# alshai/rowbowt

Hardware: AMD Instinct MI355X
Metric: reads/s (100 bp, count+locate) (higher is better)
Workload: dtype u32/u64

## Files before the change

### rowbowt_amd/csrc/k_runs.hip

```cpp
#include <type_traits>

#include "rbg_runs2_device.hpp"
#include "rbg_jump.h"

namespace rbg {
namespace {

struct PackedBits {
    const uint4 *__restrict__ cp;
    uint4 w;
    uint32_t widx, navail;
    uint64_t sr;
    __device__ __forceinline__ uint32_t next_word() {
        if (widx == 4) { w = *cp++; widx = 0; }
        const uint32_t v = w.x;
        w.x = w.y; w.y = w.z; w.z = w.w;
        ++widx;
        return v;
    }
    __device__ __forceinline__ uint32_t take(uint32_t nb) {
        if (navail < nb) { sr |= static_cast<uint64_t>(next_word()) << navail; navail += 32; }
        const uint32_t v = static_cast<uint32_t>(sr & ((uint64_t(1) << nb) - 1));
        sr >>= nb;
        navail -= nb;
        return v;
    }
};

template <bool GLDS>
__device__ __forceinline__ bool jump_probe_wave(const void *__restrict__ tab, const uint64_t nb, const bool probing, const JumpKey &key, uint32_t v[3],
                                                uint32_t &buckets, lds_byte *tile) {
    uint32_t state = probing ? kJumpNext : kJumpAbsent;
    uint64_t b = probing ? jump_home(jump_hash(key), nb) : 0u;
    uint64_t left = nb;
    while (__ballot(state == kJumpNext)) {
        const bool undecided = state == kJumpNext;
        uint32_t w[16];
        quad_fetch_issue<GLDS>(reinterpret_cast<uint64_t>(tab) + (undecided ? b : 0u) * kJumpBucketBytes, w, tile);
        quad_fetch_take<GLDS>(w, tile);
        if (undecided) {
            ++buckets;
            state = jump_bucket(w, key, v);
            b = jump_next(b, nb);
            if (--left == 0 && state == kJumpNext) state = kJumpAbsent;
        }
    }
    return state <= kJumpHit1;
}

template <typename P, bool TOEHOLD, bool PACKED = false, bool STATS = false, bool GLDS = false, bool STAGE = false>
__global__ __launch_bounds__(512, STATS ? 2 : 4) void k_find_range_runs(const DevIndex ix, const void *__restrict__ src_a,
                                                        const void *__restrict__ src_b, const uint64_t N,
                                                        uint64_t *__restrict__ lo_out, uint64_t *__restrict__ hi_out,
                                                        uint64_t *__restrict__ ss_out, unsigned long long *__restrict__ stats,
                                                        const uint32_t *__restrict__ sel, const uint32_t *__restrict__ nsel) {
    const uint64_t Neff = sel ? static_cast<uint64_t>(*nsel) : N;
    const uint8_t *__restrict__ seqs = static_cast<const uint8_t *>(src_a);
    const uint64_t *__restrict__ off = static_cast<const uint64_t *>(src_b);
    const uint4 *__restrict__ chunks = static_cast<const uint4 *>(src_a);
    const uint2 *__restrict__ meta = static_cast<const uint2 *>(src_b);
    __shared__ uint8_t s_lut[256];
    __shared__ uint8_t s_lut2[256];
    __shared__ uint8_t s_mslot[4];
    __shared__ __align__(16) unsigned char s_tile[GLDS ? 8 * kTileBytes : 16];
    __shared__ uint32_t s_codes[STAGE ? 8 * kStageWords * 64 : 1];
    for (int t = threadIdx.x; t < 256; t += blockDim.x) {
        s_lut[t] = ix.lut[t];
        s_lut2[t] = ix.nmajor ? ix.lut2[t] : 0xFFu;
    }
    RBG_RUN_SEARCH2_SHARED;
    const RunSearch2<P> S2 = stage_run_search2<P>(ix, s_tab_first, s_ent2, s_dir2, s_rec2, s_dyn);
    const uint32_t *tab_first = s_tab_first;
    lds_byte *tile = (lds_byte *)s_tile + (GLDS ? (threadIdx.x >> 6) * kTileBytes : 0u);
    if (PACKED || STAGE) {
        for (int t = threadIdx.x; t < 256; t += blockDim.x)
            if (s_lut2[t] != 0xFFu) s_mslot[s_lut2[t] & 3u] = s_lut[t];
        __syncthreads();
    }
    const uint32_t D = ix.run_ksteps, DMASK = ix.run_depth_mask | 1u;
    const uint32_t M = ix.nmajor;
    const uint32_t lane = threadIdx.x & (kWave - 1);
    lds_u32 *codes = (lds_u32 *)s_codes + (STAGE ? (threadIdx.x >> 6) * (kStageWords * 64u) + lane : 0u);
    const StageTab stage_tab{ix.stage_code[0], ix.stage_code[1], ix.stage_byte[0], ix.stage_byte[1], ix.stage_shift};
    const bool stage_on = STAGE && ix.stage_ok != 0 && M == 4;

    unsigned long long c_occ = 0, c_reads = 0;
    uint32_t c_matched = 0;
    unsigned long long st[kStatSearchN] = {0, 0, 0, 0, 0, 0, 0, 0};
    const uint64_t stride = static_cast<uint64_t>(gridDim.x) * blockDim.x;
    const uint64_t wave_first = static_cast<uint64_t>(blockIdx.x) * blockDim.x + (threadIdx.x & ~(kWave - 1));
    for (uint64_t base = wave_first; base < Neff; base += stride) {
        bool valid = base + lane < Neff;
        const uint64_t i = (sel && valid) ? static_cast<uint64_t>(sel[base + lane]) : base + lane;
        uint64_t beg = 0, p = 0;
        PackedBits bs{chunks, make_uint4(0, 0, 0, 0), 4u, 0u, 0ull};
        if (PACKED) {
            if (valid) {
                const uint2 mt = meta[i];
                if (mt.y & 0x80000000u) valid = false;
                else { p = mt.y; bs.cp = chunks + mt.x; }
            }
        } else if (valid) { beg = off[i]; p = off[i + 1]; }
        bool staged = false;
        if constexpr (STAGE && !PACKED) {
            if (stage_on && __ballot(valid && p - beg > kStageCap) == 0) {
                uint32_t nch = 0;
                const bool bad = valid && stage_read(reinterpret_cast<const uint4 *>(seqs), beg, p, stage_tab, codes, nch);
                if (STATS) st[kStChunks] += nch;
                staged = __ballot(bad) == 0;
                if (staged) { p -= beg; beg = 0; }
                else if (STATS) st[kStChunks] -= nch;
            }
        }
        auto walk = [&](auto staged_tag) __attribute__((always_inline)) {
            constexpr bool STAGED = decltype(staged_tag)::value;
            const uint64_t p_end = p;
            uint64_t p_min = p;
            const uint32_t m32 = static_cast<uint32_t>(p);
            uint64_t lo = 0, hi = ix.n - 1;
            uint64_t k = TOEHOLD ? ix.last_run_sample : 0;
            bool alive = valid;
            bool pend = false;
            uint32_t pend_d = 0, pend_rec = 0;
            uint64_t pend_e = 0;
            ByteCursor rd{reinterpret_cast<const uint4 *>(seqs), ~uint64_t(0), make_uint4(0, 0, 0, 0)};
            bool jumped = false;
            if constexpr (STAGED && sizeof(P) == 4) {
                if (ix.jump) {
                    const bool probing = valid && m32 >= ix.jump_k;
                    JumpKey key{{codes[0], codes[64], codes[128], codes[192]}};
                    jump_key_mask(key, ix.jump_k);
                    uint32_t v[3] = {0, 0, 0}, nbk = 0;
                    if (jump_probe_wave<GLDS>(ix.jump, ix.jump_buckets, probing, key, v, nbk, tile)) {
                        lo = v[0]; hi = v[1];
                        if (TOEHOLD) k = v[2] == 0xFFFFFFFFu ? ~uint64_t(0) : static_cast<uint64_t>(v[2]);
                        p -= ix.jump_k;
                        jumped = true;
                        if (STATS) st[kStSymbols] += ix.jump_k;
                    }
                    if (STATS) st[kStFtab] += nbk;
                }
            }
            if (!jumped && valid && ix.ftab_k && p - beg >= ix.ftab_k) {
                uint64_t idx = 0;
                bool all_major = true;
                PackedBits probe = bs;
                if constexpr (STAGED) {
                    const uint32_t w0 = codes[0];
                    idx = ix.ftab_k >= 16u ? w0 : (w0 & ((1u << (2u * ix.ftab_k)) - 1u));
                } else if (PACKED) {
                    idx = probe.take(2 * ix.ftab_k);
                } else {
                    uint64_t pw = 1;
                    for (uint32_t t = 1; t <= ix.ftab_k; ++t) {
                        const uint32_t mm = s_lut2[rd.at(p - t)];
                        all_major = all_major && mm != 0xFFu;
                        idx += (mm & 3u) * pw;
                        pw *= M;
                    }
                }
                uint64_t flo, fhi2, fk;
                if (STATS) { if (!STAGED) p_min = p - ix.ftab_k; if (all_major) st[kStFtab] += 1; }
                if (all_major && ftab_lookup<P>(ix, idx, flo, fhi2, fk)) {
                    if (PACKED) bs = probe;
                    lo = flo; hi = fhi2;
                    if (TOEHOLD) k = fk;
                    p -= ix.ftab_k;
                    if (STATS) st[kStSymbols] += ix.ftab_k;
                    if (hi < lo) { alive = false; p = beg; }
                }
            }
            struct Pick { uint32_t d, adv, rec; bool ok; };
            auto pick_at = [&](const uint64_t pp) __attribute__((always_inline)) -> Pick {
                Pick s{0u, 1u, 0u, true};
                if constexpr (STAGED) {
                    s.adv = pp < D ? static_cast<uint32_t>(pp) : D;
                    s.adv = 32u - static_cast<uint32_t>(__clz(DMASK & ((2u << (s.adv - 1)) - 1u)));
                    const uint32_t t0 = m32 - static_cast<uint32_t>(pp);
                    const lds_u32 *cw = codes + (t0 >> 4) * 64u;
                    const uint32_t v = __builtin_amdgcn_alignbit(cw[64], cw[0], (t0 & 15u) * 2u) & ((1u << (2u * s.adv)) - 1u);
                    s.rec = run_record(tab_first, s.adv, s.adv == 1 ? static_cast<uint32_t>(s_mslot[v]) : v);
                    s.d = s.adv - 1;
                } else if (PACKED) {
                    s.adv = pp < D ? static_cast<uint32_t>(pp) : D;
                    s.adv = 32u - static_cast<uint32_t>(__clz(DMASK & ((2u << (s.adv - 1)) - 1u)));
                    const uint32_t v = bs.take(2 * s.adv);
                    s.rec = run_record(tab_first, s.adv, s.adv == 1 ? static_cast<uint32_t>(s_mslot[v]) : v);
                    s.d = s.adv - 1;
                } else {
                    const uint64_t q = pp - 1;
                    const uint32_t c = rd.at(q);
                    if (STATS && q < p_min) p_min = q;
                    const uint32_t m0 = s_lut2[c];
                    uint32_t acc = m0;
                    if (m0 != 0xFFu) {
                        uint32_t pw = M, run_acc = m0;
    #pragma unroll 1
                        for (uint32_t t = 1; t < static_cast<uint32_t>(kMaxRunDepth); ++t) {
                            if (t >= D || q < beg + t) break;
                            const uint32_t mm = s_lut2[rd.at(q - t)];
                            if (STATS && q - t < p_min) p_min = q - t;
                            if (mm == 0xFFu) break;
                            run_acc += mm * pw;
                            pw *= M;
                            if ((DMASK >> t) & 1u) { s.adv = t + 1; acc = run_acc; }
                        }
                    }
                    if (s.adv == 1) {
                        const uint32_t slot = s_lut[c];
                        if (slot == 0xFFu || slot >= static_cast<uint32_t>(kLdsSyms)) s.ok = false;
                        else s.rec = run_record(tab_first, 1u, slot);
                    } else {
                        s.d = s.adv - 1;
                        s.rec = run_record(tab_first, s.adv, acc);
                    }
                }
                return s;
            };
            constexpr bool AHEAD = !PACKED || STAGED;
            Pick cur{0u, 1u, 0u, false};
            RunHot Rcur{0, 0};
            if (AHEAD && alive && p > beg) {
                cur = pick_at(p);
                if (cur.ok) Rcur = load_run_tab<P>(S2, cur.d, cur.rec);
            }
            while (__ballot(alive && p > beg)) {
                bool stepping = alive && p > beg;
                if (!AHEAD && stepping) {
                    cur = pick_at(p);
                    if (cur.ok) Rcur = load_run_tab<P>(S2, cur.d, cur.rec);
                }
                if (stepping && !cur.ok) { alive = false; stepping = false; }
                const uint32_t d = cur.d, adv = cur.adv, rec = cur.rec;
                const RunHot R = Rcur;
                const uint64_t p_next = p - adv;
                if (AHEAD && stepping && p_next > beg) {
                    cur = pick_at(p_next);
                    if (cur.ok) Rcur = load_run_tab<P>(S2, cur.d, cur.rec);
                }
                RunStep r;
                lane_lf2_quad<P, STATS, false, GLDS>(S2, stepping, d, rec, R, lo, hi + 1, r, st, tile);
                if (stepping) {
                    if (STATS) st[kStSymbols] += adv;
                    const uint64_t c_inside = r.c_upto - r.c_before;
                    if (c_inside == 0) {
                        alive = false;
                    } else {
                        if (TOEHOLD) {
                            if (r.inside) k = k - adv;
                            else { pend = true; pend_d = d; pend_rec = rec; pend_e = r.samp_e; k = 0; }
                        }
                        lo = r.F + r.c_before;
                        hi = lo + c_inside - 1;
                        p = p_next;
                    }
                }
            }
            if (TOEHOLD && alive && pend) {
                k += run_step_sample2<P>(ix, S2, pend_d, pend_rec, pend_e);
                if (STATS) st[kStResample] += 1;
            }
            if (STATS && !PACKED && !STAGED && p_end > p_min) st[kStChunks] += ((p_end - 1) >> 4) - (p_min >> 4) + 1;
            if (STATS && PACKED && valid) st[kStChunks] += (p_end + 63) >> 6;
            if (!alive) { lo = 1; hi = 0; k = 0; }
            if (valid) {
                lo_out[i] = lo;
                hi_out[i] = hi;
                if (TOEHOLD) ss_out[i] = k;
                c_reads += 1;
                if (alive) { c_matched += 1; c_occ += hi - lo + 1; }
            }
        };
        if (STAGE && staged) walk(std::integral_constant<bool, STAGE>{}); else walk(std::false_type{});
    }
    c_reads = wave_sum(c_reads);
    const unsigned long long w_matched = wave_sum(static_cast<unsigned long long>(c_matched));
    c_occ = wave_sum(c_occ);
    if (lane == 0 && c_reads) {
        atomicAdd(&ix.counters[0], c_reads);
        if (w_matched) atomicAdd(&ix.counters[1], w_matched);
        if (c_occ) atomicAdd(&ix.counters[2], c_occ);
    }
    if (STATS) {
#pragma unroll
        for (int t = 0; t < kStatSearchN; ++t) {
            const unsigned long long v = wave_sum(st[t]);
            if (lane == 0 && v) atomicAdd(&stats[t], v);
        }
    }
}

template <typename P> struct ChunkR { static constexpr int v = 8; };
__device__ __forceinline__ uint64_t locus_toehold_r(const DevIndex &ix, const uint64_t key, const uint64_t *__restrict__ k, const uint64_t i) {
    if (key == ~uint64_t(0)) return k[i];
    const uint32_t low = ix.order_lowbits, db = ix.order_dbits;
    const uint64_t doc = (key >> low) & ((uint64_t(1) << db) - 1u);
    return ix.order_docs[doc] + (((key >> (db + low)) << low) | (key & ((uint64_t(1) << low) - 1u)));
}

template <typename P, typename OUT = uint64_t, bool STATS = false, bool SUB = false, bool HI8 = false>
__global__ __launch_bounds__(256, 4) void k_locate_fill_runs2(const DevIndex ix, const uint64_t *__restrict__ lo,
                                                          const uint64_t *__restrict__ hi, const uint64_t *__restrict__ k,
                                                          const uint64_t N, const uint64_t max_hits,
                                                          const uint64_t *__restrict__ loc_off, OUT *__restrict__ locs,
                                                          const uint64_t *__restrict__ sub, const uint32_t *__restrict__ order,
                                                          const uint64_t *__restrict__ skeys, unsigned long long *__restrict__ stats) {
    constexpr int kChunkR = ChunkR<P>::v;
    constexpr bool RING = true;
    using Stage = ChainStage<P, kChunkR, SUB, RING, HI8>;
    __shared__ Stage S;
    const uint64_t out_elem0 = reinterpret_cast<uintptr_t>(locs) / sizeof(OUT);
    const int wv = threadIdx.x >> 6, lane = threadIdx.x & (kWave - 1);
    unsigned long long c_locs = 0;
    unsigned long long st_phi = 0, st_ent = 0, st_chains = 0;
    const uint64_t n = ix.n;
    const uint64_t stride = static_cast<uint64_t>(gridDim.x) * blockDim.x;
    for (uint64_t base = static_cast<uint64_t>(blockIdx.x) * blockDim.x + wv * kWave; base < N; base += stride) {
        const uint64_t j = base + lane;
        uint64_t i = j;
        if (order && j < N) i = order[j];
        uint64_t occ = 0, k1 = 0, dst = 0;
        if (i < N && j < N) {
            dst = loc_off[i];
            if (skeys) {
                if (ix.order_docs) k1 = locus_toehold_r(ix, skeys[j], k, i);
                else if (sizeof(P) == 4) { const uint32_t k32 = reinterpret_cast<const uint32_t *>(skeys)[j]; k1 = k32 == 0xFFFFFFFFu ? k[i] : k32; }
                else k1 = skeys[j];
                occ = loc_off[i + 1] - dst;
            } else {
                const uint64_t l = lo[i], h = hi[i];
                occ = h >= l ? h - l + 1 : 0;
                if (occ > max_hits) occ = max_hits;
                k1 = k[i];
            }
        }
        const uint64_t minus = (SUB && i < N && j < N) ? sub[i] : 0;
        const uint32_t a = (RING && occ) ? static_cast<uint32_t>((out_elem0 + dst) & static_cast<uint64_t>(kChunkR - 1)) : 0u;
        S.dst[wv][lane] = dst - a;
        if (SUB) S.minus[wv][lane] = minus;
        const bool off_text = Stage::kSentinel && k1 >= n;
        if (off_text && occ) locs[dst] = static_cast<OUT>(k1 - minus);
        c_locs += occ;
        if (STATS && occ) st_chains += 1;
        uint64_t wmax = occ + a;
#pragma unroll
        for (int o = kWave / 2; o > 0; o >>= 1) {
            const uint64_t other = __shfl_xor(wmax, o, kWave);
            wmax = other > wmax ? other : wmax;
        }
        for (uint64_t t0 = 0; t0 < wmax; t0 += kChunkR) {
            const uint32_t cnt = chain_round_count<kChunkR>(occ, t0);
            S.bounds[wv][lane] = chain_window_bounds<kChunkR>(occ, a, t0);
#pragma unroll 1
            for (int e = 0; e < kChunkR; ++e) {
                const bool mine = static_cast<uint32_t>(e) < cnt;
                if (mine && (e || t0)) {
                    uint64_t s;
                    if (k1 >= n) {
                        s = (ix.phi_last_base + (k1 - ix.phi_last_pos)) % n;
                    } else {
                        bool found;
                        uint64_t val;
                        uint32_t ents, rounds;
                        lane_phi<P>(ix, k1, found, val, ents, rounds);
                        if (STATS) { st_phi += 1; st_ent += ents + 7u * rounds; }
                        s = found ? val : ix.phi_last_base + k1 + 1;
                        if (s >= n) s -= n;
                    }
                    k1 = s;
                }
                if (mine) chain_put(S, wv, lane, a + static_cast<uint32_t>(t0) + e, k1, e == 0 && t0 == 0 && off_text);
            }
            wave_lds_sync();
            chain_flush(S, wv, lane, t0, locs);
            wave_lds_sync();
        }
        wave_lds_sync();
    }
    c_locs = wave_sum(c_locs);
    if (lane == 0 && c_locs) atomicAdd(&ix.counters[3], c_locs);
    if (STATS) {
        st_phi = wave_sum(st_phi);
        st_ent = wave_sum(st_ent);
        st_chains = wave_sum(st_chains);
        if (lane == 0) {
            if (st_phi) atomicAdd(&stats[kLsPhiSteps], st_phi);
            if (st_ent) atomicAdd(&stats[kLsPhiOvf], st_ent);
            if (st_chains) atomicAdd(&stats[kLsChains], st_chains);
            if (c_locs) atomicAdd(&stats[kLsLocs], c_locs);
        }
    }
}

}

int launch_find_range_runs_impl(const DevIndex &ix, const LaunchCfg &cfg, const void *src_a, const void *src_b, uint64_t N,
                                uint64_t *lo, uint64_t *hi, uint64_t *ssamp, void *stream, bool packed, unsigned long long *stats,
                                const uint32_t *sel = nullptr, const uint32_t *nsel = nullptr) {
    if (N == 0) return 0;
    hipStream_t st = static_cast<hipStream_t>(stream);
    const size_t lds = run_search2_lds(ix);
    static const bool glds = [] { const char *e = std::getenv("RBG_REC_FETCH"); return !(e && std::strcmp(e, "quad") == 0); }();
    static const bool stage = [] { const char *e = std::getenv("RBG_STAGE_READS"); return !(e && e[0] == '0'); }();
    LaunchCfg c = cfg;
    c.block_threads = 512;
    c.max_blocks = cfg.max_blocks > 0 ? std::max(1, cfg.max_blocks / 2) : 256 * 16;
    const dim3 grid(sel ? std::min(grid_for(c, N), 256) : grid_for(c, N)), block(512);
#define RBG_LAUNCH_FRR1(PT, TOE, PK, STS, GL, SG)                                                      \
    do {                                                                                               \
        auto kern = k_find_range_runs<PT, TOE, PK, STS, GL, SG>;                                       \
        raise_lds(kern, lds, (GL ? 8 * kTileBytes : 0) + (SG ? 8 * kStageWaveBytes : 0));             \
        hipLaunchKernelGGL(kern, grid, block, lds, st, ix, src_a, src_b, N, lo, hi, ssamp, stats, sel, nsel);     \
    } while (0)
#define RBG_LAUNCH_FRR(PT, TOE, PK, STS)                                                               \
    do {                                                                                               \
        if (glds && stage && !PK && !sel) RBG_LAUNCH_FRR1(PT, TOE, false, STS, true, true);            \
        else if (glds) RBG_LAUNCH_FRR1(PT, TOE, PK, STS, true, false);                                 \
        else RBG_LAUNCH_FRR1(PT, TOE, PK, STS, false, false);                                          \
    } while (0)
#define RBG_LAUNCH_FRR2(PT, TOE)                                                                       \
    do {                                                                                               \
        if (stats) { if (packed) return static_cast<int>(hipErrorNotSupported); RBG_LAUNCH_FRR(PT, TOE, false, true); } \
        else if (packed) RBG_LAUNCH_FRR(PT, TOE, true, false);                                         \
        else RBG_LAUNCH_FRR(PT, TOE, false, false);                                                    \
    } while (0)
    if (ix.pos_bytes == 4) {
        if (ssamp) RBG_LAUNCH_FRR2(uint32_t, true); else RBG_LAUNCH_FRR2(uint32_t, false);
    } else {
        if (ssamp) RBG_LAUNCH_FRR2(uint64_t, true); else RBG_LAUNCH_FRR2(uint64_t, false);
    }
#undef RBG_LAUNCH_FRR2
#undef RBG_LAUNCH_FRR
#undef RBG_LAUNCH_FRR1
    return static_cast<int>(hipGetLastError());
}

int launch_find_range_runs(const DevIndex &ix, const LaunchCfg &cfg, const uint8_t *seqs, const uint64_t *off, uint64_t N,
                           uint64_t *lo, uint64_t *hi, uint64_t *ssamp, void *stream, unsigned long long *stats) {
    return launch_find_range_runs_impl(ix, cfg, seqs, off, N, lo, hi, ssamp, stream, false, stats);
}

int launch_find_range_runs_sel(const DevIndex &ix, const LaunchCfg &cfg, const uint8_t *seqs, const uint64_t *off, uint64_t N, uint64_t *lo,
                               uint64_t *hi, uint64_t *ssamp, const uint32_t *sel, const uint32_t *nsel, void *stream) {
    return launch_find_range_runs_impl(ix, cfg, seqs, off, N, lo, hi, ssamp, stream, false, nullptr, sel, nsel);
}

int launch_find_range_runs_packed(const DevIndex &ix, const LaunchCfg &cfg, const uint2 *meta, const uint4 *chunks, uint64_t N,
                                  uint64_t *lo, uint64_t *hi, uint64_t *ssamp, void *stream) {
    return launch_find_range_runs_impl(ix, cfg, chunks, meta, N, lo, hi, ssamp, stream, true, nullptr);
}

int launch_locate_fill_runs(const DevIndex &ix, const LaunchCfg &cfg, const uint64_t *lo, const uint64_t *hi, const uint64_t *k,
                            uint64_t N, uint64_t max_hits, const uint64_t *loc_off, uint64_t *locs, const uint64_t *sub,
                            const void *order, const uint64_t *skeys, void *stream, unsigned long long *stats, uint32_t *locs32) {
    if (N == 0) return 0;
    if ((stats || locs32) && sub) return static_cast<int>(hipErrorInvalidValue);
    hipStream_t st = static_cast<hipStream_t>(stream);
    const dim3 grid(grid_for(cfg, N)), block(256);
    const uint32_t *perm = static_cast<const uint32_t *>(order);
    const bool hi8 = ix.pos_bytes == 8 && ix.n < kChainHi8Limit && chain_hi8_enabled();
#define RBG_LAUNCH_LFR2(PT, OUT, STS, SB, DST) \
    do { \
        if (sizeof(PT) == 8 && hi8) hipLaunchKernelGGL((k_locate_fill_runs2<PT, OUT, STS, SB, sizeof(PT) == 8>), grid, block, 0, st, ix, lo, hi, k, N, max_hits, loc_off, DST, sub, perm, skeys, stats); \
        else hipLaunchKernelGGL((k_locate_fill_runs2<PT, OUT, STS, SB, false>), grid, block, 0, st, ix, lo, hi, k, N, max_hits, loc_off, DST, sub, perm, skeys, stats); \
    } while (0)
    if (locs32) {
        if (ix.pos_bytes != 4) return static_cast<int>(hipErrorInvalidValue);
        RBG_LAUNCH_LFR2(uint32_t, uint32_t, false, false, locs32);
    } else if (stats) {
        if (ix.pos_bytes == 4) RBG_LAUNCH_LFR2(uint32_t, uint64_t, true, false, locs); else RBG_LAUNCH_LFR2(uint64_t, uint64_t, true, false, locs);
    } else if (sub) {
        if (ix.pos_bytes == 4) RBG_LAUNCH_LFR2(uint32_t, uint64_t, false, true, locs); else RBG_LAUNCH_LFR2(uint64_t, uint64_t, false, true, locs);
    } else if (ix.pos_bytes == 4) {
        RBG_LAUNCH_LFR2(uint32_t, uint64_t, false, false, locs);
    } else {
        RBG_LAUNCH_LFR2(uint64_t, uint64_t, false, false, locs);
    }
#undef RBG_LAUNCH_LFR2
    return static_cast<int>(hipGetLastError());
}

}
```

Before: 2.192 billion.

## Park jump-table misses and finish them in a compacted tail kernel

Reads whose jump-table probe misses are no longer walked inside the main wave. They are marked in lo_out, and a second kernel scans the output, compacts the parked read indices into per-wave LDS queues, and walks them with full waves. This targets divergence, where a few slow reads stall a whole wave of fast jump hits. The cost is an extra launch and a full scan of lo_out, and the tail kernel runs smaller blocks at lower occupancy.

```diff
diff --git a/rowbowt_amd/csrc/k_runs.hip b/rowbowt_amd/csrc/k_runs.hip
--- a/rowbowt_amd/csrc/k_runs.hip
+++ b/rowbowt_amd/csrc/k_runs.hip
@@ -2,6 +2,7 @@
 
 #include "rbg_runs2_device.hpp"
 #include "rbg_jump.h"
+#include "rbg_park.h"
 
 namespace rbg {
 namespace {
@@ -48,12 +49,15 @@
     return state <= kJumpHit1;
 }
 
-template <typename P, bool TOEHOLD, bool PACKED = false, bool STATS = false, bool GLDS = false, bool STAGE = false>
-__global__ __launch_bounds__(512, STATS ? 2 : 4) void k_find_range_runs(const DevIndex ix, const void *__restrict__ src_a,
+template <typename P, bool TOEHOLD, bool PACKED = false, bool STATS = false, bool GLDS = false, bool STAGE = false, bool TAIL = false>
+__global__ __launch_bounds__(TAIL ? 256 : 512, TAIL ? (STATS ? 2 : 3) : (STATS ? 2 : 4)) void k_find_range_runs(const DevIndex ix, const void *__restrict__ src_a,
                                                         const void *__restrict__ src_b, const uint64_t N,
                                                         uint64_t *__restrict__ lo_out, uint64_t *__restrict__ hi_out,
                                                         uint64_t *__restrict__ ss_out, unsigned long long *__restrict__ stats,
-                                                        const uint32_t *__restrict__ sel, const uint32_t *__restrict__ nsel) {
+                                                        const uint32_t *__restrict__ sel, const uint32_t *__restrict__ nsel,
+                                                        const uint32_t park) {
+    static_assert(!TAIL || (STAGE && GLDS && !PACKED && sizeof(P) == 4), "the tail walks staged reads of an index with 4-byte positions");
+    constexpr uint32_t kWavesWG = TAIL ? 4 : 8;
     const uint64_t Neff = sel ? static_cast<uint64_t>(*nsel) : N;
     const uint8_t *__restrict__ seqs = static_cast<const uint8_t *>(src_a);
     const uint64_t *__restrict__ off = static_cast<const uint64_t *>(src_b);
@@ -62,8 +66,9 @@
     __shared__ uint8_t s_lut[256];
     __shared__ uint8_t s_lut2[256];
     __shared__ uint8_t s_mslot[4];
-    __shared__ __align__(16) unsigned char s_tile[GLDS ? 8 * kTileBytes : 16];
-    __shared__ uint32_t s_codes[STAGE ? 8 * kStageWords * 64 : 1];
+    __shared__ __align__(16) unsigned char s_tile[GLDS ? kWavesWG * kTileBytes : 16];
+    __shared__ uint32_t s_codes[STAGE ? kWavesWG * kStageWords * 64 : 1];
+    __shared__ uint32_t s_queue[TAIL ? kWavesWG * kParkQueueWords : 1];
     for (int t = threadIdx.x; t < 256; t += blockDim.x) {
         s_lut[t] = ix.lut[t];
         s_lut2[t] = ix.nmajor ? ix.lut2[t] : 0xFFu;
@@ -89,9 +94,7 @@
     unsigned long long st[kStatSearchN] = {0, 0, 0, 0, 0, 0, 0, 0};
     const uint64_t stride = static_cast<uint64_t>(gridDim.x) * blockDim.x;
     const uint64_t wave_first = static_cast<uint64_t>(blockIdx.x) * blockDim.x + (threadIdx.x & ~(kWave - 1));
-    for (uint64_t base = wave_first; base < Neff; base += stride) {
-        bool valid = base + lane < Neff;
-        const uint64_t i = (sel && valid) ? static_cast<uint64_t>(sel[base + lane]) : base + lane;
+    auto iter = [&](bool valid, const uint64_t i) __attribute__((always_inline)) {
         uint64_t beg = 0, p = 0;
         PackedBits bs{chunks, make_uint4(0, 0, 0, 0), 4u, 0u, 0ull};
         if (PACKED) {
@@ -106,10 +109,10 @@
             if (stage_on && __ballot(valid && p - beg > kStageCap) == 0) {
                 uint32_t nch = 0;
                 const bool bad = valid && stage_read(reinterpret_cast<const uint4 *>(seqs), beg, p, stage_tab, codes, nch);
-                if (STATS) st[kStChunks] += nch;
+                if (STATS && !TAIL) st[kStChunks] += nch;
                 staged = __ballot(bad) == 0;
                 if (staged) { p -= beg; beg = 0; }
-                else if (STATS) st[kStChunks] -= nch;
+                else if (STATS && !TAIL) st[kStChunks] -= nch;
             }
         }
         auto walk = [&](auto staged_tag) __attribute__((always_inline)) {
@@ -124,8 +127,8 @@
             uint32_t pend_d = 0, pend_rec = 0;
             uint64_t pend_e = 0;
             ByteCursor rd{reinterpret_cast<const uint4 *>(seqs), ~uint64_t(0), make_uint4(0, 0, 0, 0)};
-            bool jumped = false;
-            if constexpr (STAGED && sizeof(P) == 4) {
+            bool jumped = false, parked = false;
+            if constexpr (STAGED && sizeof(P) == 4 && !TAIL) {
                 if (ix.jump) {
                     const bool probing = valid && m32 >= ix.jump_k;
                     JumpKey key{{codes[0], codes[64], codes[128], codes[192]}};
@@ -137,11 +140,14 @@
                         p -= ix.jump_k;
                         jumped = true;
                         if (STATS) st[kStSymbols] += ix.jump_k;
+                    } else if (park && probing) {
+                        parked = true;
+                        alive = false;
                     }
                     if (STATS) st[kStFtab] += nbk;
                 }
             }
-            if (!jumped && valid && ix.ftab_k && p - beg >= ix.ftab_k) {
+            if (!jumped && !parked && valid && ix.ftab_k && p - beg >= ix.ftab_k) {
                 uint64_t idx = 0;
                 bool all_major = true;
                 PackedBits probe = bs;
@@ -263,7 +269,9 @@
             if (STATS && !PACKED && !STAGED && p_end > p_min) st[kStChunks] += ((p_end - 1) >> 4) - (p_min >> 4) + 1;
             if (STATS && PACKED && valid) st[kStChunks] += (p_end + 63) >> 6;
             if (!alive) { lo = 1; hi = 0; k = 0; }
-            if (valid) {
+            if (parked) {
+                lo_out[i] = kParkMark;
+            } else if (valid) {
                 lo_out[i] = lo;
                 hi_out[i] = hi;
                 if (TOEHOLD) ss_out[i] = k;
@@ -272,6 +280,44 @@
             }
         };
         if (STAGE && staged) walk(std::integral_constant<bool, STAGE>{}); else walk(std::false_type{});
+    };
+    if constexpr (TAIL) {
+        lds_u32 *queue = (lds_u32 *)s_queue + (threadIdx.x >> 6) * kParkQueueWords;
+        const uint64_t W = static_cast<uint64_t>(gridDim.x) * kWavesWG, w = static_cast<uint64_t>(blockIdx.x) * kWavesWG + (threadIdx.x >> 6);
+        const uint64_t r0 = park_first(N, W, w), r1 = park_end(N, W, w);
+        uint64_t pos = r0;
+        uint32_t qn = 0;
+        for (;;) {
+            while (park_scan_more(qn, pos, r1)) {
+                uint64_t v[kParkScanChunks];
+#pragma unroll
+                for (uint32_t c = 0; c < kParkScanChunks; ++c) {
+                    const uint64_t at = pos + c * kParkWave + lane;
+                    v[c] = at < r1 ? lo_out[at] : 0u;
+                }
+#pragma unroll
+                for (uint32_t c = 0; c < kParkScanChunks; ++c) {
+                    const bool marked = v[c] == kParkMark;
+                    const uint64_t mask = __ballot(marked);
+                    if (marked) queue[park_slot(qn, mask, lane)] = static_cast<uint32_t>(pos - r0) + c * kParkWave + lane;
+                    qn += park_count(mask);
+                }
+                pos += kParkScan;
+            }
+            if (qn == 0) break;
+            wave_lds_sync();
+            const uint32_t first = park_take_first(qn);
+            const bool valid = lane < park_take(qn);
+            const uint64_t i = r0 + (valid ? queue[first + lane] : 0u);
+            qn = first;
+            wave_lds_sync();
+            iter(valid, i);
+        }
+    } else {
+        for (uint64_t base = wave_first; base < Neff; base += stride) {
+            const bool valid = base + lane < Neff;
+            iter(valid, (sel && valid) ? static_cast<uint64_t>(sel[base + lane]) : base + lane);
+        }
     }
     c_reads = wave_sum(c_reads);
     const unsigned long long w_matched = wave_sum(static_cast<unsigned long long>(c_matched));
@@ -406,15 +452,31 @@
     c.block_threads = 512;
     c.max_blocks = cfg.max_blocks > 0 ? std::max(1, cfg.max_blocks / 2) : 256 * 16;
     const dim3 grid(sel ? std::min(grid_for(c, N), 256) : grid_for(c, N)), block(512);
+    constexpr size_t kTailStatic = 4 * (kTileBytes + kStageWaveBytes + kParkQueueWords * sizeof(uint32_t));
+    const bool tail_fits = lds + kTailStatic + 1024 <= 160 * 1024;
+    const uint32_t park = (!sel && !packed && glds && stage && ix.pos_bytes == 4 && ix.jump && ix.stage_ok && ix.nmajor == 4 &&
+                           N < kParkMaxReads && tail_fits) ? 1u : 0u;
+    const uint64_t tail_cus = cfg.max_blocks > 0 ? std::max(1, cfg.max_blocks / 32) : 256;
+    const uint64_t tail_per_cu = std::min<uint64_t>(3, std::max<uint64_t>(1, 160 * 1024 / (lds + kTailStatic + 1024)));
+    const dim3 tail_grid(static_cast<unsigned>(std::min<uint64_t>(tail_cus * tail_per_cu, (N + 16 * kParkScan - 1) / (16 * kParkScan)))), tail_block(256);
 #define RBG_LAUNCH_FRR1(PT, TOE, PK, STS, GL, SG)                                                      \
     do {                                                                                               \
         auto kern = k_find_range_runs<PT, TOE, PK, STS, GL, SG>;                                       \
         raise_lds(kern, lds, (GL ? 8 * kTileBytes : 0) + (SG ? 8 * kStageWaveBytes : 0));             \
-        hipLaunchKernelGGL(kern, grid, block, lds, st, ix, src_a, src_b, N, lo, hi, ssamp, stats, sel, nsel);     \
+        hipLaunchKernelGGL(kern, grid, block, lds, st, ix, src_a, src_b, N, lo, hi, ssamp, stats, sel, nsel, (SG && sizeof(PT) == 4) ? park : 0u); \
+    } while (0)
+#define RBG_LAUNCH_FRR_TAIL(TOE, STS)                                                                  \
+    do {                                                                                               \
+        auto tail = k_find_range_runs<uint32_t, TOE, false, STS, true, true, true>;                    \
+        raise_lds(tail, lds, kTailStatic);                                                             \
+        hipLaunchKernelGGL(tail, tail_grid, tail_block, lds, st, ix, src_a, src_b, N, lo, hi, ssamp, stats, sel, nsel, 0u); \
     } while (0)
 #define RBG_LAUNCH_FRR(PT, TOE, PK, STS)                                                               \
     do {                                                                                               \
-        if (glds && stage && !PK && !sel) RBG_LAUNCH_FRR1(PT, TOE, false, STS, true, true);            \
+        if (glds && stage && !PK && !sel) {                                                            \
+            RBG_LAUNCH_FRR1(PT, TOE, false, STS, true, true);                                          \
+            if (sizeof(PT) == 4 && park) RBG_LAUNCH_FRR_TAIL(TOE, STS);                                \
+        }                                                                                              \
         else if (glds) RBG_LAUNCH_FRR1(PT, TOE, PK, STS, true, false);                                 \
         else RBG_LAUNCH_FRR1(PT, TOE, PK, STS, false, false);                                          \
     } while (0)
@@ -431,6 +493,7 @@
     }
 #undef RBG_LAUNCH_FRR2
 #undef RBG_LAUNCH_FRR
+#undef RBG_LAUNCH_FRR_TAIL
 #undef RBG_LAUNCH_FRR1
     return static_cast<int>(hipGetLastError());
 }
diff --git a/rowbowt_amd/csrc/rbg_park.h b/rowbowt_amd/csrc/rbg_park.h
--- /dev/null
+++ b/rowbowt_amd/csrc/rbg_park.h
@@ -0,0 +1,52 @@
+#pragma once
+
+#include <cstdint>
+
+#if defined(__HIPCC__)
+#define RBG_PARK_HD __host__ __device__ __forceinline__
+#else
+#define RBG_PARK_HD inline
+#endif
+
+namespace rbg {
+
+constexpr uint64_t kParkMark = ~uint64_t(0);
+constexpr uint32_t kParkWave = 64;
+constexpr uint32_t kParkScanChunks = 4;
+constexpr uint32_t kParkScan = kParkScanChunks * kParkWave;
+constexpr uint32_t kParkQueueCap = (kParkWave - 1) + kParkScan;
+constexpr uint32_t kParkQueueWords = kParkQueueCap + 1;
+constexpr uint64_t kParkMaxReads = uint64_t(1) << 32;
+
+RBG_PARK_HD uint64_t park_span(uint64_t N, uint64_t W) {
+    const uint64_t per = (N + W - 1) / W;
+    return (per + kParkScan - 1) / kParkScan * kParkScan;
+}
+RBG_PARK_HD uint64_t park_first(uint64_t N, uint64_t W, uint64_t w) {
+    const uint64_t r0 = w * park_span(N, W);
+    return r0 < N ? r0 : N;
+}
+RBG_PARK_HD uint64_t park_end(uint64_t N, uint64_t W, uint64_t w) {
+    const uint64_t r1 = (w + 1) * park_span(N, W);
+    return r1 < N ? r1 : N;
+}
+RBG_PARK_HD bool park_scan_more(uint32_t qn, uint64_t pos, uint64_t r1) { return qn < kParkWave && pos < r1; }
+RBG_PARK_HD uint32_t park_slot(uint32_t qn, uint64_t mask, uint32_t lane) {
+    const uint64_t below = mask & ((uint64_t(1) << lane) - 1u);
+#if defined(__HIP_DEVICE_COMPILE__)
+    return qn + static_cast<uint32_t>(__popcll(below));
+#else
+    return qn + static_cast<uint32_t>(__builtin_popcountll(below));
+#endif
+}
+RBG_PARK_HD uint32_t park_count(uint64_t mask) {
+#if defined(__HIP_DEVICE_COMPILE__)
+    return static_cast<uint32_t>(__popcll(mask));
+#else
+    return static_cast<uint32_t>(__builtin_popcountll(mask));
+#endif
+}
+RBG_PARK_HD uint32_t park_take(uint32_t qn) { return qn < kParkWave ? qn : kParkWave; }
+RBG_PARK_HD uint32_t park_take_first(uint32_t qn) { return qn - park_take(qn); }
+
+}
```

After: 2.113 billion. -3.6%, worse.
